# AislingGui/cst_captioning

Measured on AMD Instinct MI355X. Metric: SCST training captions/sec (whole node), MSR-VTT LSTM-attn at 1/2/4/8 MI355X, higher is better.
Workload: dtype bf16; 1 GPU; model=CaptionModel concat LSTM-512 (resnet+c3d+mfcc+category, V=10509, L=30), global_batch=1280, videos_per_gpu=64, seq_per_img=20, seq_len=30, parallelism=dp1, impl=hip, reward=gpu, mode=scst, params=20888845, dedupe_greedy=1, cuda_graph=1, grad_wire=fp32

## Files before the change

csrc/bindings.cpp:

```cpp
#include <torch/extension.h>

#include "engine.h"
#include "host/cider_host.h"
#include "host/metric_host.h"
#include "launchers.h"

namespace cst {

template <class T>
static at::Tensor to_tensor(const std::vector<T>& v, at::ScalarType st) {
  at::Tensor t = at::empty({(int64_t)v.size()}, at::TensorOptions().dtype(st));
  if (!v.empty()) std::memcpy(t.data_ptr(), v.data(), v.size() * sizeof(T));
  return t;
}

static std::map<std::string, at::Tensor> cider_build_tables(at::Tensor labels, at::Tensor start,
                                                            at::Tensor end, at::Tensor df_keys,
                                                            at::Tensor df_vals,
                                                            double log_ref_len, int64_t use_eos) {
  TORCH_CHECK(!labels.is_cuda(), "host builder takes CPU tensors");
  labels = labels.contiguous().to(at::kLong);
  start = start.contiguous().to(at::kLong);
  end = end.contiguous().to(at::kLong);
  df_keys = df_keys.contiguous().to(at::kLong);
// ... 254 lines not shown
          return py::cast(cst::reward_mix_score(hyps, hyp_video, cider_tables, tables,
                                                log_ref_len, use_eos, *weights));
        }
        TORCH_CHECK(tables.has_value(), "metric_score: tables must be given");
        TORCH_CHECK(!weights.has_value() && !cider_tables.has_value(),
                    "metric_score: weights / cider_tables go with metric mix only");
        return py::cast(cst::metric_score(metric, hyps, hyp_video, *tables, use_eos, exclude));
      },
      py::arg("metric"), py::arg("hyps"), py::arg("hyp_video"), py::arg("tables"),
      py::arg("use_eos"), py::arg("exclude") = py::none(), py::arg("cider_tables") = py::none(),
      py::arg("log_ref_len") = 0.0, py::arg("weights") = py::none(), py::arg("group") = 0,
      "Bleu_4 | ROUGE_L sentence scores on the GPU, or their weighted mix with CIDEr-D "
      "(metric mix; group = G >= 2: every row against the others of its pool of G); one "
      "launch, capturable");
  m.def(
      "metric_score_cpu",
      [](const std::string& metric, at::Tensor hyps, at::Tensor hyp_video,
         c10::optional<std::map<std::string, at::Tensor>> tables, int64_t use_eos,
         c10::optional<at::Tensor> exclude,
         c10::optional<std::map<std::string, at::Tensor>> cider_tables, double log_ref_len,
         c10::optional<std::vector<double>> weights, int64_t group) -> py::object {
        if (group != 0) {
          TORCH_CHECK(metric == "mix",
                      "metric_score_cpu: peer mode (group > 0) is metric mix, got ", metric);
          TORCH_CHECK(weights.has_value(), "metric_score_cpu: metric mix needs weights");
          TORCH_CHECK(!(exclude.has_value() && exclude->defined()),
                      "metric_score_cpu: peer mode (group > 0) takes no exclude");
          return py::cast(cst::peer_mix_score_cpu(hyps, cider_tables, log_ref_len, use_eos,
                                                  *weights, group));
        }
        TORCH_CHECK(!weights.has_value() && !cider_tables.has_value(),
                    "metric_score_cpu: weights / cider_tables go with peer mode (metric mix, "
                    "group > 0) only");
        TORCH_CHECK(tables.has_value(), "metric_score_cpu: tables must be given");
        return py::cast(cst::metric_score_cpu(metric, hyps, hyp_video, *tables, use_eos, exclude));
      },
      py::arg("metric"), py::arg("hyps"), py::arg("hyp_video"), py::arg("tables"),
      py::arg("use_eos"), py::arg("exclude") = py::none(), py::arg("cider_tables") = py::none(),
      py::arg("log_ref_len") = 0.0, py::arg("weights") = py::none(), py::arg("group") = 0);
  m.def("flat_adam_step", &cst::flat_adam_step, py::arg("p"), py::arg("g"), py::arg("m"),
        py::arg("v"), py::arg("partials"), py::arg("scal"), py::arg("skip"), py::arg("hyper"),
        py::arg("b1"), py::arg("b2"), py::arg("eps"), py::arg("clip"), py::arg("gscale"),
        py::arg("phase"), py::arg("shadow_meta"), py::arg("shadow_dst"),
        py::arg("ema") = py::none(), py::arg("ema_decay") = 0.0);
  m.def("refresh_shadows", &cst::refresh_shadows, py::arg("p"), py::arg("shadow_meta"),
        py::arg("shadow_dst"), py::arg("swap_with") = py::none());
  m.def("vocab_fwd_bench", &cst::vocab_fwd_bench);
  m.def("vgrad_colsum_bench", &cst::vgrad_colsum_bench);
  m.def("token_sort_bench", &cst::token_sort_bench);
  m.def("att_bench", &cst::att_bench);
  m.def("token_sort", &cst::token_sort);
  m.def("token_group_sum", &cst::token_group_sum);
  m.def("vocab_select", &cst::vocab_select);
  m.def("decode_step_test", &cst::decode_step_test);
  m.def("gemm_bf16_tuned", &cst::gemm_bf16_tuned, py::arg("out"), py::arg("a"), py::arg("ta"),
        py::arg("b"), py::arg("tb"), py::arg("n_cand") = 24);
  m.def("gemm_bf16_tuned_batched", &cst::gemm_bf16_tuned_batched, py::arg("out"), py::arg("a"),
        py::arg("ta"), py::arg("b"), py::arg("tb"), py::arg("n_cand") = 24);
  m.def("gemm_tuned_timings", &cst::gemm_tuned_timings);
  m.def("gemm_tuned_choices", &cst::gemm_tuned_choices);
  m.def("set_grad_events", &cst::set_grad_events);
  m.def("grad_event_wait", &cst::grad_event_wait);
  m.def("grad_event_record", &cst::grad_event_record);
  m.def("grad_event_count", &cst::grad_event_count);
  m.def("set_poll_bound", &cst::set_poll_bound,
        "polls of a bounded cross-workgroup wait before it gives up (tests: 0)");
  m.def("set_bwd_loop", &cst::set_bwd_loop,
        "reverse LSTM loop: 1 one persistent launch, row-read form (default); 2 persistent, "
        "K-split team GEMM; 0 one launch per step");
  m.def("lstm_bwd_loop_bench", &cst::lstm_bwd_loop_bench, py::arg("R"), py::arg("H"), py::arg("T"),
        py::arg("iters"), py::arg("phases"), py::arg("dbg") = 0,
        "persistent reverse loop alone on random operands: us per launch (+ phase stamps)");
  m.def("set_att_fuse", &cst::set_att_fuse,
        "attention backward fused into the reverse step (true, default) or a launch per step");
  m.def("device_errors", &cst::device_errors,
        "failed cross-workgroup hand-offs counted on the device (synchronous read)");
  m.def("reset_device_errors", &cst::reset_device_errors);
  m.def("att_mfma_fwd", &cst::att_mfma_fwd, py::arg("h"), py::arg("wq"), py::arg("P"),
        py::arg("wa"), py::arg("ba"), py::arg("gv"), py::arg("whole") = -1);
  m.def("beam_search", &cst::beam_search);
  m.def("featpool_forward", &cst::featpool_forward, py::arg("xs"), py::arg("ws"), py::arg("bs"),
        py::arg("drop_p"), py::arg("rng"), py::arg("idx") = py::none(), py::arg("C") = 1);
  m.def("featpool_forward16", &cst::featpool_forward16, py::arg("xs"), py::arg("ws"),
        py::arg("bs"), py::arg("drop_p"), py::arg("rng"), py::arg("idx") = py::none(),
        py::arg("C") = 1);
  m.def("scst_loss_forward", &cst::scst_loss_forward);
  m.def("cst_loss_forward", &cst::cst_loss_forward, py::arg("seq"), py::arg("lp"),
        py::arg("scores"), py::arg("bref"), py::arg("S"), py::arg("k"), py::arg("objective") = 0,
        py::arg("alpha") = 1.0, py::arg("cost_scale") = 1.0);
  m.def("scst_loss_backward", &cst::scst_loss_backward, py::arg("seq"), py::arg("reward"),
        py::arg("out"), py::arg("dloss"), py::arg("row_weight") = py::none());
  m.def("xe_loss_forward", &cst::xe_loss_forward);
  m.def("xe_loss_backward", &cst::xe_loss_backward);
  m.def("featpool_backward", &cst::featpool_backward, py::arg("dout"), py::arg("out"),
        py::arg("xs"), py::arg("ws"), py::arg("drop_p"), py::arg("outs"),
        py::arg("idx") = py::none(), py::arg("C") = 1);
  m.def("set_stamp_base", &cst::set_stamp_base);
  m.def("stamp_buffer", &cst::stamp_buffer);
  m.def("stamp_now", &cst::stamp_now);
  m.def("busy_copy", &cst::busy_copy,
        "stand-in for a collective's kernel: copying workgroups for a given time");
  m.def("wall_clock_khz", &cst::wall_clock_khz);
  m.def("vocab_x", &cst::vocab_x);
  m.def("att_mfma_phases", &cst::att_mfma_phases);
  m.def("wgrad_tn", &cst::wgrad_tn);
  m.def("wgrad_tn_colsum", &cst::wgrad_tn_colsum);
  m.def("wgrad_tn_rows", &cst::wgrad_tn_rows);
// ... 10 lines not shown
```

csrc/decoder_forward.cpp:

```cpp
#include "engine_internal.h"

namespace cst {
namespace {

struct Rollout {
  const at::Tensor &wx, &emb, &ptab, &whh, &wlog, &blog, &vgate;
  const int64_t vgate_div;
  const at::Tensor &labels, &bos;
  const int64_t R, T;
  const std::vector<int64_t>& modes;
  const double ss_prob, drop_p, temperature;
  const at::Tensor& rng;
  const bool save, want_xe, use_counts, use_unfinished;
  const std::vector<at::Tensor>& att;
  const int64_t cell;
  const std::vector<at::Tensor>&state0, &up;
  const bool store_exp, xe_rows;
  const c10::optional<at::Tensor>& lab_idx;
  bool has_att = false, have_labels = false, have_idx = false;
  int64_t H4 = 0, H = 0, E = 0, V = 0, L = 0, n_steps = 0, NL = 1;
  const uint16_t* PTAB = nullptr;
  AttOperands ao;
  UpperLayers upl;
  InitState s0;
// ... 221 lines not shown
    at::Tensor tgt_all = labels.narrow(1, 1, n_steps).t().contiguous();
    at::Tensor gx = at::empty({n_steps, R}, f32);
    stamp(STAMP_FWD_BEGIN, st);
    launch_lstm_step_fwd(LAB, L, PTAB, nullptr, nullptr, VG, VDIV, (int)R, (int)H, WHH,
                         h_buf(0, 0), c_buf(0, 0), hd_buf(0, 0), (int)H, (float)drop_p, RNG,
                         key(0, 0), gates_buf(0, 0), st, nullptr, (int)cell);
    stamp(STAMP_FWD_STEP0, st);
    for (int64_t t = 0; t < n_steps; ++t) {
      const bool next = t + 1 < n_steps;
      XeCell xc{};
      if (next)
        xc = XeCell{LAB + (t + 1), L, PTAB, c_buf(0, t), h_buf(0, t + 1), c_buf(0, t + 1),
                    hd_buf(0, t + 1), gates_buf(0, t + 1), (float)drop_p, key(0, t + 1),
                    (int)cell};
      char* pt = reinterpret_cast<char*>(part_all.data_ptr()) + t * pstep;
      launch_vocab_lstm_xe(hd_buf(0, t), (int)R, (int)H, W, blog.data_ptr<float>(), (int)V,
                           reinterpret_cast<uint16_t*>(logits16[t].data_ptr()), ldl, pt,
                           tgt_all.data_ptr<int64_t>() + t * R, RNG, h_buf(0, t), WHH, VG, VDIV,
                           next ? &xc : nullptr, st);
    }
    launch_vocab_combine(part_all.data_ptr(), n_vt, (int)(n_steps * R), lse.data_ptr<float>(),
                         nullptr, 0, nullptr, 0, gx.data_ptr<float>(), 1, nullptr, 0, SEL_GT_H,
                         0.f, RNG, 0, nullptr, 0, nullptr, st, nullptr, (int)R);
    at::Tensor gxt = gx.t();
    g_xe.copy_(gxt);
    g_sel.copy_(gxt.narrow(1, 0, T - 1));
    seq.copy_(labels.narrow(1, 1, T - 1));
    stamp(STAMP_FWD_END, st);
    return {seq, g_sel, g_xe, lse, logits16, HDs[0], Gs[0], Cs[0], Hs[0]};
  }

  std::vector<at::Tensor> run_steps() {
    const int64_t Bv = ao.Bv, C = ao.C, A = ao.A;
    stamp(STAMP_FWD_BEGIN, st);
    if (has_att) run_att(0);
    launch_lstm_step_fwd(have_labels ? LABR : TokRows(bos.data_ptr<int64_t>()), have_labels ? L : 1,
                         PTAB,
                         state0.empty() ? nullptr : reinterpret_cast<uint16_t*>(h0.data_ptr()),
                         state0.empty() ? nullptr : c0.data_ptr<float>(), VG, VDIV, (int)R, (int)H, WHH, h_buf(0, 0),
                         c_buf(0, 0), hd_buf(0, 0), (int)H, (float)drop_p, RNG, key(0, 0),
                         gates_buf(0, 0), st, nullptr, (int)cell, &sinit);
    for (int64_t l = 1; l < NL; ++l) upper_step(l, 0);
    bool conv_join = false;
    for (int64_t t = 0; t < n_steps; ++t) {
      const bool next = t + 1 < n_steps;
      uint16_t* hd = hd_buf(NL - 1, t);
      const uint16_t* vin = hd ? hd : h_buf(NL - 1, t);
      const bool choose = t < T - 1;
      const int mode = choose ? (int)modes[t] : SEL_GT_H;
      const int do_sample = choose && (mode == SEL_SAMPLE_H || mode == SEL_SS_H);
      const bool exp_t = save && store_exp && t > 0;
      const int vflags = do_sample | ((choose && mode == SEL_GREEDY_H) ? 2 : 0) | (exp_t ? 16 : 0);
      const TokRows tgt = (have_labels && t + 1 < L) ? LABR.col(t + 1) : TokRows();
      at::Tensor q_next;
      if (has_att && next) q_next = save ? q_all[t + 1] : q_tmp;
      AttMfmaArgs am{};
      if (att_mfma && next)
        am = AttMfmaArgs{h_buf(0, t), WHH + H4 * H, ao.pre.data_ptr<float>(), ao.wa.data_ptr<float>(),
                         ao.ba.data_ptr<float>(), reinterpret_cast<const uint16_t*>(gv16.data_ptr()),
                         (int)H, (int)A, (int)C, ao.CPAD, (int)H4, (int)vgate_div, (int)Bv,
                         reinterpret_cast<uint16_t*>(vg16.data_ptr()),
                         save ? alpha_all[t + 1].data_ptr<float>() : nullptr,
                         save ? q_next.data_ptr<float>() : nullptr, att_ep.data_ptr<float>(),
                         att_cnt.data_ptr<int>(),
                         save ? reinterpret_cast<uint16_t*>(u_all[t + 1].data_ptr()) : nullptr};
      if (att_mfma && next) am.whole = att_mfma_whole_default((int)C, (int)H);
      const bool q_tiles = has_att && !att_mfma;
      const int n_vt = launch_vocab_lstm_fwd(
          vin, (int)H, (int)R, (int)H, W, blog.data_ptr<float>(), (int)V,
          save ? reinterpret_cast<uint16_t*>(logits16[t].data_ptr()) : nullptr, ldl, part.data_ptr(),
          tgt, L, vflags, inv_temp, RNG, (int)t, h_buf(0, t), WHH, has_att ? nullptr : VG, VDIV,
          next ? reinterpret_cast<float*>(pre.data_ptr()) : nullptr, st, q_tiles ? (int)A : 0,
          q_tiles && next ? q_next.data_ptr<float>() : nullptr,
          exp_t ? lse[t - 1].data_ptr<float>() : nullptr, att_mfma && next ? &am : nullptr,
          pre16 ? 1 : 0);
      if (q_tiles && next)
        launch_att_fwd(ao.gv.data_ptr<float>(), ao.pre.data_ptr<float>(), q_next.data_ptr<float>(),
                       nullptr, ao.wa.data_ptr<float>(), ao.ba.data_ptr<float>(), (int)Bv,
                       (int)vgate_div, (int)C, (int)A, (int)H4, pre.data_ptr<float>(),
                       save ? alpha_all[t + 1].data_ptr<float>() : nullptr, st, 1,
                       ao.per_frame);
      CellLaunch cl{};
      if (next) {
        TORCH_CHECK(choose, "internal: a next step needs a chosen token");
        cl = CellLaunch{pre.data_ptr(), PTAB, c_buf(0, t), c_buf(0, t + 1),
                        h_buf(0, t + 1), hd_buf(0, t + 1), (int)H, gates_buf(0, t + 1), (int)H,
                        (float)drop_p, key(0, t + 1), (int)cell,
                        att_mfma ? reinterpret_cast<const uint16_t*>(vg16.data_ptr()) : nullptr,
                        pre16 ? 1 : 0};
      }
      launch_vocab_combine(part.data_ptr(), n_vt, (int)R, lse[t].data_ptr<float>(),
                             choose ? seq.data_ptr<int64_t>() + t : nullptr, T - 1,
                             choose ? g_sel.data_ptr<float>() + t : nullptr, T - 1,
                             want_xe ? g_xe.data_ptr<float>() + t : nullptr, T, tgt, L, mode,
                             (float)ss_prob, RNG, (int)t,
                             use_counts ? counts.data_ptr<int>() : nullptr, (int)(t + 1),
                             use_unfinished ? unfinished.data_ptr<uint8_t>() : nullptr, st,
                             next ? &cl : nullptr);
      if (save && store_exp && t == 0) {
        DeviceAux& aux = device_aux((int)wx.device().index());
        const hipStream_t cs = aux.side[1].stream();
        fork(aux.fwd_ev[0], st, cs);
        launch_vocab_exp_convert(reinterpret_cast<uint16_t*>(logits16[0].data_ptr()), ldl, (int)V,
                                 (int)R, lse[0].data_ptr<float>(), cs);
        (void)hipEventRecord(aux.fwd_ev[1], cs);
        conv_join = true;
      }
      if (next)
        for (int64_t l = 1; l < NL; ++l) upper_step(l, t + 1);
      if (t == 0) stamp(STAMP_FWD_STEP0, st);
    }
    if (conv_join)
      (void)hipStreamWaitEvent(st, device_aux((int)wx.device().index()).fwd_ev[1], 0);
    stamp(STAMP_FWD_END, st);
    std::vector<at::Tensor> out = {seq, g_sel, want_xe ? g_xe : at::Tensor(), lse};
    if (save) {
      out.push_back(logits16);
      out.push_back(HDs[NL - 1]);
      out.push_back(Gs[0]);
      out.push_back(Cs[0]);
      out.push_back(Hs[0]);
      if (has_att) {
        out.push_back(alpha_all);
        out.push_back(q_all);
// ... 36 lines not shown
```

csrc/dev_entries.cpp:

```cpp
#include "engine_internal.h"

namespace cst {

double lstm_bwd_loop_bench(int64_t R, int64_t H, int64_t T, int64_t iters, at::Tensor phases,
                           int64_t dbg) {
  TORCH_CHECK(lstm_bwd_loop_ok((int)R, (int)H, (int)T), "lstm_bwd_loop_bench: unsupported shape");
  auto dev = at::Device(at::kCUDA, at::hip::getCurrentHIPStream().device_index());
  auto f32 = at::TensorOptions().dtype(at::kFloat).device(dev);
  auto b16 = at::TensorOptions().dtype(at::kBFloat16).device(dev);
  at::Tensor dG = at::empty({T, R, 4 * H}, b16);
  at::Tensor whhT = (at::randn({H, 4 * H}, f32) * 0.05).to(at::kBFloat16);
  at::Tensor dh = at::randn({T, R, H}, f32) * 0.01;
  at::Tensor gates = at::rand({T, R, 4 * H}, f32).to(at::kBFloat16);
  at::Tensor c_all = at::randn({T, R, H}, f32);
  at::Tensor dc = at::empty({R, H}, f32);
  at::Tensor rng = at::zeros({2}, at::TensorOptions().dtype(at::kInt).device(dev));
  BwdLoopArgs la{};
  la.dG = reinterpret_cast<uint16_t*>(dG.data_ptr());
  la.whhT = reinterpret_cast<const uint16_t*>(whhT.data_ptr());
  la.dh = dh.data_ptr<float>();
  la.gates = reinterpret_cast<const uint16_t*>(gates.data_ptr());
  la.c_all = c_all.data_ptr<float>();
  la.dc_out = dc.data_ptr<float>();
  la.R = (int)R;
// ... 268 lines not shown
  const int vdiv = (int)(R / Bv), CP = C <= 8 ? 8 : 16;
  TORCH_CHECK(att_mfma_fwd_ok(vdiv, (int)C, (int)A, (int)H, 0), "att_mfma: unsupported shape");
  at::Tensor gv16 = at::zeros({Bv, 4 * H, CP}, h.options());
  gv16.narrow(2, 0, C).copy_(gv.transpose(1, 2));
  at::Tensor vg = at::empty({R, 4 * H}, h.options());
  at::Tensor alpha = at::empty({R, C}, P.options()), q = at::empty({R, A}, P.options());
  at::Tensor ep = at::empty({Bv, A / 64, 32, CP}, P.options());
  at::Tensor cnt = at::zeros({Bv}, P.options().dtype(at::kInt));
  AttMfmaArgs a{reinterpret_cast<const uint16_t*>(h.data_ptr()),
                reinterpret_cast<const uint16_t*>(wq.data_ptr()), P.data_ptr<float>(),
                wa.data_ptr<float>(), ba.data_ptr<float>(),
                reinterpret_cast<const uint16_t*>(gv16.data_ptr()), (int)H, (int)A, (int)C, CP,
                (int)(4 * H), vdiv, (int)Bv, reinterpret_cast<uint16_t*>(vg.data_ptr()),
                alpha.data_ptr<float>(), q.data_ptr<float>(), ep.data_ptr<float>(),
                cnt.data_ptr<int>()};
  a.whole = whole < 0 ? att_mfma_whole_default((int)C, (int)H) : (whole != 0 ? 1 : 0);
  launch_att_mfma_fwd(a, cur_stream());
  return {vg, alpha, q};
}

std::vector<at::Tensor> vocab_select(at::Tensor hd, at::Tensor wlog, at::Tensor blog,
                                     at::Tensor rng, int64_t mode, double temperature,
                                     int64_t step) {
  check_cuda(hd, "hd");
  check_cuda(wlog, "wlog");
  TORCH_CHECK(hd.scalar_type() == at::kBFloat16 && wlog.scalar_type() == at::kBFloat16 &&
                  blog.scalar_type() == at::kFloat, "bf16 hd / W, fp32 bias");
  TORCH_CHECK(mode == SEL_SAMPLE_H || mode == SEL_GREEDY_H, "mode: 1 sample, 2 greedy");
  const int64_t R = hd.size(0), H = hd.size(1), V = wlog.size(0);
  TORCH_CHECK(H % 64 == 0 && wlog.size(1) == H && blog.numel() == V, "shapes");
  auto dev = hd.device();
  const int n_vt = vocab_num_tiles((int)V);
  at::Tensor part = at::empty({(int64_t)n_vt * R * vocab_partial_bytes() / 4},
                              at::TensorOptions().dtype(at::kFloat).device(dev));
  at::Tensor tok = at::zeros({R, 1}, at::TensorOptions().dtype(at::kLong).device(dev));
  at::Tensor lse = at::empty({R}, at::TensorOptions().dtype(at::kFloat).device(dev));
  hipStream_t st = cur_stream();
  launch_vocab_fwd(reinterpret_cast<const uint16_t*>(hd.data_ptr()), (int)H, (int)R, (int)H,
                   reinterpret_cast<const uint16_t*>(wlog.data_ptr()), blog.data_ptr<float>(),
                   (int)V, nullptr, 0, part.data_ptr(), nullptr, 0, mode == SEL_SAMPLE_H ? 1 : 2,
                   (float)(1.0 / temperature), rng_ptr(rng), (int)step, st);
  launch_vocab_combine(part.data_ptr(), n_vt, (int)R, lse.data_ptr<float>(),
                       tok.data_ptr<int64_t>(), 1, nullptr, 0, nullptr, 0, nullptr, 0, (int)mode,
                       0.f, rng_ptr(rng), (int)step, nullptr, 0, nullptr, st);
  return {tok.view({R}), lse};
}

std::vector<at::Tensor> decode_step_test(at::Tensor hd, at::Tensor h, at::Tensor wlog,
                                         at::Tensor blog, at::Tensor whh, at::Tensor vgate,
                                         int64_t vdiv, at::Tensor tgt, at::Tensor eoff,
                                         int64_t save, int64_t mode, int64_t step, at::Tensor rng,
                                         at::Tensor ptab, at::Tensor c_prev, double drop_p,
                                         int64_t cell, int64_t eos, at::Tensor unfinished,
                                         double ss_prob) {
  check_cuda(hd, "hd");
  check_cuda(wlog, "wlog");
  const int64_t R = hd.size(0), H = hd.size(1), V = wlog.size(0);
  TORCH_CHECK(hd.scalar_type() == at::kBFloat16 && wlog.scalar_type() == at::kBFloat16 &&
                  hd.is_contiguous() && wlog.is_contiguous() && wlog.size(1) == H &&
                  blog.scalar_type() == at::kFloat && blog.numel() == V, "hd / wlog / blog");
  const bool lstm = whh.defined() && whh.numel() > 0;
  if (lstm)
    TORCH_CHECK(h.scalar_type() == at::kBFloat16 && h.is_contiguous() && h.sizes() == hd.sizes() &&
                    whh.scalar_type() == at::kBFloat16 && whh.is_contiguous() &&
                    whh.size(0) == 4 * H && whh.size(1) == H, "h / whh");
  const bool has_vg = vgate.defined() && vgate.numel() > 0;
  if (has_vg)
    TORCH_CHECK(vgate.scalar_type() == at::kFloat && vgate.is_contiguous() &&
                    vgate.size(0) * vdiv == R && vgate.size(1) == 4 * H, "vgate (R / vdiv, 4H)");
  const bool has_tgt = tgt.defined() && tgt.numel() > 0;
  if (has_tgt) TORCH_CHECK(tgt.scalar_type() == at::kLong && tgt.numel() == R, "tgt (R) int64");
  if (save == 2)
    TORCH_CHECK(eoff.defined() && eoff.scalar_type() == at::kFloat && eoff.numel() == R, "eoff (R)");
  const bool do_cell = ptab.defined() && ptab.numel() > 0;
  if (do_cell) {
    TORCH_CHECK(lstm, "the cell needs the recurrent part");
    check_cuda(ptab, "ptab");
    check_cuda(c_prev, "c_prev");
    TORCH_CHECK(ptab.scalar_type() == at::kHalf && ptab.size(0) == V && ptab.size(1) == 4 * H &&
                    c_prev.scalar_type() == at::kFloat && c_prev.numel() == R * H,
                "ptab (V, 4H) fp16 / c_prev (R, H) fp32");
  }
  const bool has_unf = unfinished.defined() && unfinished.numel() > 0;
  if (has_unf)
    TORCH_CHECK(unfinished.is_cuda() && unfinished.scalar_type() == at::kByte &&
                    unfinished.numel() == R, "unfinished (R) uint8");
  auto dev = hd.device();
  auto f32 = at::TensorOptions().dtype(at::kFloat).device(dev);
  auto bf = at::TensorOptions().dtype(at::kBFloat16).device(dev);
  const int64_t ldl = (V + 63) / 64 * 64;
  at::Tensor part = at::empty({(int64_t)vocab_part_slots((int)V) * R * vocab_partial_bytes() / 4}, f32);
  at::Tensor saved = save ? at::zeros({R, ldl}, at::TensorOptions()
                                                    .dtype(save == 2 ? at::kBFloat16 : at::kHalf)
                                                    .device(dev))
                          : at::Tensor();
  at::Tensor pre = lstm ? at::zeros({R, 4 * H}, f32) : at::Tensor();
  at::Tensor lse = at::empty({R}, f32), gsel = at::zeros({R}, f32), gxe = at::zeros({R}, f32);
  at::Tensor tok = at::zeros({R}, at::TensorOptions().dtype(at::kLong).device(dev));
  at::Tensor h_out, c_out, hdrop, gates;
  if (do_cell) {
    h_out = at::zeros({R, H}, bf);
    c_out = at::zeros({R, H}, f32);
    hdrop = at::zeros({R, H}, bf);
    gates = at::zeros({R, 4 * H}, bf);
  }
  const int cps = combine_count_ints_per_step();
  at::Tensor counts = at::zeros({3 * cps}, at::TensorOptions().dtype(at::kInt).device(dev));
  if (eos == 1) counts.narrow(0, cps, 1).fill_(1);
  int* CNT = eos ? counts.data_ptr<int>() : nullptr;
  hipStream_t st = cur_stream();
  const int flags = (mode == SEL_SAMPLE_H || mode == SEL_SS_H ? 1 : 0) |
                    (mode == SEL_GREEDY_H ? 2 : 0) | (save == 2 ? 16 : 0);
  const int64_t* TG = has_tgt ? tgt.data_ptr<int64_t>() : nullptr;
  uint8_t* UNF = has_unf ? unfinished.data_ptr<uint8_t>() : nullptr;
  const int n = launch_vocab_lstm_fwd(
      reinterpret_cast<const uint16_t*>(hd.data_ptr()), (int)H, (int)R, (int)H,
      reinterpret_cast<const uint16_t*>(wlog.data_ptr()), blog.data_ptr<float>(), (int)V,
      save ? reinterpret_cast<uint16_t*>(saved.data_ptr()) : nullptr, ldl, part.data_ptr(), TG, 1,
      flags, 1.f, rng_ptr(rng), (int)step,
      lstm ? reinterpret_cast<const uint16_t*>(h.data_ptr()) : nullptr,
      lstm ? reinterpret_cast<const uint16_t*>(whh.data_ptr()) : nullptr,
      has_vg ? vgate.data_ptr<float>() : nullptr, (int)vdiv, lstm ? pre.data_ptr<float>() : nullptr,
      st, 0, nullptr, save == 2 ? eoff.data_ptr<float>() : nullptr, nullptr);
  CellLaunch cl{};
  if (do_cell)
    cl = CellLaunch{pre.data_ptr<float>(), reinterpret_cast<const uint16_t*>(ptab.data_ptr()),
                    c_prev.data_ptr<float>(), c_out.data_ptr<float>(),
                    reinterpret_cast<uint16_t*>(h_out.data_ptr()),
                    reinterpret_cast<uint16_t*>(hdrop.data_ptr()), (int)H,
                    reinterpret_cast<uint16_t*>(gates.data_ptr()), (int)H, (float)drop_p,
                    (int)step + 1, (int)cell, nullptr, 0};
  launch_vocab_combine(part.data_ptr(), n, (int)R, lse.data_ptr<float>(), tok.data_ptr<int64_t>(),
                       1, gsel.data_ptr<float>(), 1, has_tgt ? gxe.data_ptr<float>() : nullptr, 1,
                       TG, 1, (int)mode, (float)ss_prob, rng_ptr(rng), (int)step, CNT, 2, UNF, st,
                       do_cell ? &cl : nullptr);
  return {lse, tok, gsel, gxe, saved, pre, at::full({1}, n, at::TensorOptions().dtype(at::kLong)),
          h_out, c_out, hdrop, gates, counts};
}

std::vector<at::Tensor> token_sort(at::Tensor toks, int64_t V) {
  check_cuda(toks, "toks");
  TORCH_CHECK(toks.scalar_type() == at::kLong, "int64 token ids");
  const int64_t N = toks.numel();
  auto i32 = at::TensorOptions().dtype(at::kInt).device(toks.device());
  at::Tensor ws = at::empty({2 * V + 1}, i32), stok = at::empty({N}, i32), srow = at::empty({N}, i32);
  launch_token_sort(toks.data_ptr<int64_t>(), (int)N, (int)V, ws.data_ptr<int>(),
                    stok.data_ptr<int>(), srow.data_ptr<int>(), cur_stream());
  return {stok, srow};
}

at::Tensor token_group_sum(at::Tensor x, at::Tensor toks, int64_t V) {
  check_cuda(toks, "toks");
  TORCH_CHECK(x.is_cuda() && x.scalar_type() == at::kBFloat16 && x.dim() == 2 &&
                  x.stride(1) == 1 && x.stride(0) >= x.size(1) &&
                  reinterpret_cast<uintptr_t>(x.data_ptr()) % 16 == 0,
              "x: (N, C) bf16, unit column stride, 16-byte aligned");
  TORCH_CHECK(toks.scalar_type() == at::kLong && toks.numel() == x.size(0), "toks: (N) int64");
  const int64_t N = toks.numel(), C = x.size(1);
  auto i32 = at::TensorOptions().dtype(at::kInt).device(toks.device());
  at::Tensor ws = at::empty({2 * V + 1}, i32), stok = at::empty({N}, i32), srow = at::empty({N}, i32);
  at::Tensor S = at::empty({V, C}, x.options());
  at::Tensor S64 = at::empty({V, C}, x.options().dtype(at::kDouble));
  hipStream_t st = cur_stream();
  launch_token_sort(toks.data_ptr<int64_t>(), (int)N, (int)V, ws.data_ptr<int>(),
                    stok.data_ptr<int>(), srow.data_ptr<int>(), st);
  launch_token_long_zero(ws.data_ptr<int>(), (int)V, (int)C, S64.data_ptr<double>(), st);
  launch_token_group_sum(reinterpret_cast<const uint16_t*>(x.data_ptr()), (int)C, x.stride(0),
                         stok.data_ptr<int>(), srow.data_ptr<int>(), (int)N, ws.data_ptr<int>(),
                         (int)V, reinterpret_cast<uint16_t*>(S.data_ptr()), S64.data_ptr<double>(),
                         st);
  return S;
}

std::vector<at::Tensor> vgrad_fold(at::Tensor E, at::Tensor lse, at::Tensor y_sel,
                                   at::Tensor dg_sel, at::Tensor labels, at::Tensor dg_xe,
                                   int64_t V, int64_t zero_off, at::Tensor hd, at::Tensor wlog,
                                   at::Tensor blog, at::Tensor fix_total, bool forward_x,
                                   at::Tensor X) {
  check_cuda(E, "E");
  check_cuda(lse, "lse");
  TORCH_CHECK(E.scalar_type() == at::kBFloat16 && E.dim() == 3, "vgrad_fold: E (n, R, ldl) bf16");
  const int64_t n = E.size(0), R = E.size(1), ldl = E.size(2), NR = n * R;
  TORCH_CHECK(NR > 0 && V > 0 && V <= ldl && lse.scalar_type() == at::kFloat && lse.dim() == 2 &&
                  lse.size(0) == n && lse.size(1) == R,
              "vgrad_fold: V <= ldl, lse (n, R) fp32");
  auto in_vocab = [&](const at::Tensor& t) { return t.max().item<int64_t>() < V; };
  const bool has_sel = dg_sel.defined() && dg_sel.numel() > 0;
  const bool has_xe = dg_xe.defined() && dg_xe.numel() > 0;
  int64_t T_sel = 0;
  if (has_sel) {
// ... 128 lines not shown
```

csrc/engine.h:

```cpp
#pragma once
#include <torch/extension.h>

#include <map>
#include <string>
#include <vector>

namespace cst {

std::vector<at::Tensor> decoder_forward(at::Tensor wx, at::Tensor emb, at::Tensor ptab,
                                        at::Tensor whh, at::Tensor wlog,
                                        at::Tensor blog, at::Tensor vgate, int64_t vgate_div,
                                        at::Tensor labels, at::Tensor bos, int64_t R, int64_t T,
                                        std::vector<int64_t> modes, double ss_prob,
                                        double drop_p, double temperature, at::Tensor rng,
                                        bool save, bool want_xe, bool use_counts,
                                        bool use_unfinished, std::vector<at::Tensor> att,
                                        int64_t cell, std::vector<at::Tensor> state0,
                                        std::vector<at::Tensor> up, bool store_exp,
                                        bool xe_rows, c10::optional<at::Tensor> lab_idx);
std::vector<at::Tensor> decoder_backward(at::Tensor wx, at::Tensor wlog, at::Tensor emb,
                                         at::Tensor lse, at::Tensor logits16,
                                         at::Tensor hdrop_all, at::Tensor gates_all,
                                         at::Tensor c_all, at::Tensor h_all, at::Tensor seq,
                                         at::Tensor labels, at::Tensor toks, at::Tensor dg_sel,
// ... 57 lines not shown
std::vector<at::Tensor> xe_loss_forward(at::Tensor labels, at::Tensor lp, int64_t off);
at::Tensor xe_loss_backward(at::Tensor cnt, at::Tensor out, at::Tensor dloss, int64_t T);
at::Tensor scst_loss_backward(at::Tensor seq, at::Tensor reward, at::Tensor out,
                              at::Tensor dloss, c10::optional<at::Tensor> row_weight);
at::Tensor cider_score(at::Tensor hyps, at::Tensor hyp_video, std::map<std::string, at::Tensor> t,
                       double log_ref_len, int64_t use_eos, bool clipped,
                       c10::optional<at::Tensor> exclude, int64_t group);
at::Tensor bleu_stats(at::Tensor hyps, at::Tensor hyp_video, std::map<std::string, at::Tensor> t);
std::vector<at::Tensor> meteor_stats(at::Tensor hyps, at::Tensor hyp_video,
                                     std::map<std::string, at::Tensor> t, at::Tensor stem_ids,
                                     c10::optional<at::Tensor> exclude);
at::Tensor metric_score(const std::string& metric, at::Tensor hyps, at::Tensor hyp_video,
                        std::map<std::string, at::Tensor> t, int64_t use_eos,
                        c10::optional<at::Tensor> exclude);
std::vector<at::Tensor> reward_mix_score(
    at::Tensor hyps, at::Tensor hyp_video,
    c10::optional<std::map<std::string, at::Tensor>> cider_tables,
    c10::optional<std::map<std::string, at::Tensor>> sent_tables, double log_ref_len,
    int64_t use_eos, std::vector<double> weights);
std::vector<at::Tensor> peer_mix_score(at::Tensor hyps,
                                       c10::optional<std::map<std::string, at::Tensor>> df,
                                       double log_ref_len, int64_t use_eos,
                                       std::vector<double> weights, int64_t group);
at::Tensor flat_adam_step(at::Tensor p, at::Tensor g, at::Tensor m, at::Tensor v,
                          at::Tensor partials, at::Tensor scal, at::Tensor skip, at::Tensor hyper,
                          double b1, double b2, double eps, double clip, double gscale,
                          int64_t phase, at::Tensor shadow_meta,
                          std::vector<at::Tensor> shadow_dst, c10::optional<at::Tensor> ema,
                          double ema_decay);
void refresh_shadows(at::Tensor p, at::Tensor shadow_meta, std::vector<at::Tensor> shadow_dst,
                     c10::optional<at::Tensor> swap_with);

double lstm_bwd_loop_bench(int64_t R, int64_t H, int64_t T, int64_t iters, at::Tensor phases,
                           int64_t dbg);
double vocab_fwd_bench(at::Tensor hd, at::Tensor wlog, at::Tensor blog, at::Tensor tgt,
                       int64_t flags, bool save, int64_t iters, int64_t variant);
double vgrad_colsum_bench(at::Tensor E, at::Tensor alpha, int64_t V, int64_t iters);
double token_sort_bench(at::Tensor toks, int64_t V, int64_t iters);
double att_bench(at::Tensor gv, at::Tensor P, at::Tensor q, at::Tensor wa, at::Tensor ba,
                 int64_t R, int64_t which, int64_t iters);
at::Tensor att_mfma_phases(at::Tensor gv, at::Tensor P, at::Tensor wa, at::Tensor ba, int64_t R);
std::vector<at::Tensor> att_mfma_fwd(at::Tensor h, at::Tensor wq, at::Tensor P, at::Tensor wa,
                                     at::Tensor ba, at::Tensor gv,
                                     int64_t whole);
std::vector<at::Tensor> vocab_select(at::Tensor hd, at::Tensor wlog, at::Tensor blog,
                                     at::Tensor rng, int64_t mode, double temperature,
                                     int64_t step);
std::vector<at::Tensor> decode_step_test(at::Tensor hd, at::Tensor h, at::Tensor wlog,
                                         at::Tensor blog, at::Tensor whh, at::Tensor vgate,
                                         int64_t vdiv, at::Tensor tgt, at::Tensor eoff,
                                         int64_t save, int64_t mode, int64_t step, at::Tensor rng,
                                         at::Tensor ptab, at::Tensor c_prev, double drop_p,
                                         int64_t cell, int64_t eos, at::Tensor unfinished,
                                         double ss_prob);
std::vector<at::Tensor> token_sort(at::Tensor toks, int64_t V);
at::Tensor token_group_sum(at::Tensor x, at::Tensor toks, int64_t V);
std::vector<at::Tensor> vgrad_fold(at::Tensor E, at::Tensor lse, at::Tensor y_sel,
                                   at::Tensor dg_sel, at::Tensor labels, at::Tensor dg_xe,
                                   int64_t V, int64_t zero_off, at::Tensor hd, at::Tensor wlog,
                                   at::Tensor blog, at::Tensor fix_total, bool forward_x,
                                   at::Tensor X);
at::Tensor vgrad_rows(at::Tensor alpha, at::Tensor hd, int64_t ldhs, at::Tensor dhd);
at::Tensor vgrad_colsum(at::Tensor E, at::Tensor alpha, int64_t V);
at::Tensor video_gate_grad(at::Tensor dG, int64_t vdiv, int64_t G4);
at::Tensor wgrad_tn(at::Tensor A, at::Tensor B, int64_t M, int64_t N, int64_t K);
void wgrad_tn_rows(at::Tensor A, at::Tensor B, int64_t M, int64_t N, int64_t K, at::Tensor out,
                   at::Tensor rmap);
std::vector<at::Tensor> wgrad_tn_colsum(at::Tensor A, at::Tensor B, at::Tensor al, int64_t M,
                                        int64_t N, int64_t K);
void busy_copy(at::Tensor buf, int64_t blocks, double us, int64_t stream);

}
```

csrc/kernels/vocab.hip:

```cpp
#include "gemm_tile.h"
#include "lstm_gemm.h"
#include "att_mfma.h"
#include "vocab_common.h"
#include "../launchers.h"

namespace cst {

constexpr int VT_V = 128;
constexpr int EXP_STAGE_LD = VT_V + 8;
__host__ __device__ constexpr int exp_stage_off(int BN) { return 4 * BN * 32; }
__host__ __device__ constexpr int epilogue_lds_bytes(int BN) {
  return exp_stage_off(BN) + BN * EXP_STAGE_LD * 2;
}
struct GroupStat {
  float m, s, zkey, zlogit;
  int zidx, xidx;
  float xt, pad;
};

#define VOCAB_TR_PARAMS                                                                     \
  const uint16_t *__restrict__ hd, int ldh, int R, int H, const uint16_t *__restrict__ W,    \
      const float *__restrict__ bias, int V, uint16_t *__restrict__ logits16, int64_t ldl,   \
      VocabPartial *__restrict__ part, TokRows tgt, int64_t tgt_stride,                     \
      int flags, float inv_temp, const uint32_t *__restrict__ rng, int step,                 \
      const float *__restrict__ eoff
#define VOCAB_TR_ARGS \
  hd, ldh, R, H, W, bias, V, logits16, ldl, part, tgt, tgt_stride, flags, inv_temp, rng, step, eoff

template <int BN, int STAGES, bool TOPK = false>
__device__ __forceinline__ void vocab_tr_block(int bid, char* lds, VOCAB_TR_PARAMS) {
  using TL = Tile<VT_V, BN, STAGES>;
  constexpr int TM = TL::TM, TN = TL::TN;
  static_assert(TM == 2, "lane owns 32 vocab entries per row");
  const int n_vt = (V + VT_V - 1) / VT_V, n_rt = (R + BN - 1) / BN;
  const int b = xcd_remap(bid, n_vt * n_rt);
  const int vt = b / n_rt, rt = b % n_rt;
  const int v0 = vt * VT_V, r0 = rt * BN;
  const int nk = H / 64;
  const int lane = threadIdx.x & 63, w = threadIdx.x >> 6, wr = w >> 1, wc = w & 1;
  const int half = lane >> 5;
  const int vb = v0 + wr * TL::WM + 4 * half;

  float pb[TM][16];
#pragma unroll
  for (int i = 0; i < TM; ++i)
#pragma unroll
    for (int q = 0; q < 4; ++q) {
      const int v = vb + 32 * i + 8 * q;
      if (v + 4 <= V) {
        const float4 x = *reinterpret_cast<const float4*>(bias + v);
        pb[i][4 * q] = x.x, pb[i][4 * q + 1] = x.y, pb[i][4 * q + 2] = x.z, pb[i][4 * q + 3] = x.w;
      } else {
#pragma unroll
        for (int e = 0; e < 4; ++e) pb[i][4 * q + e] = v + e < V ? bias[v + e] : -INFINITY;
      }
    }
  int tg[TN];
  float ec[TN];
#pragma unroll
  for (int j = 0; j < TN; ++j) {
    const int r = min(r0 + wc * TL::WN + 32 * j + (lane & 31), R - 1);
    tg[j] = tgt.p != nullptr ? (int)tgt.at(r, tgt_stride) : -1;
    ec[j] = eoff != nullptr ? eoff[r] : 0.f;
  }

  f32x16 acc[TM][TN];
  {
    DmaSrc<VT_V / 32> a;
    DmaSrc<BN / 32> bsrc;
    a.r0 = a.r1 = make_rsrc(W, (int64_t)V * H * 2);
    a.ksplit = nk;
#pragma unroll
    for (int i = 0; i < VT_V / 32; ++i) {
      const int row = dma_row(w, i, lane);
      a.voff0[i] = min(v0 + row, V - 1) * H * 2 + dma_chunk(row, lane) * 16;
      a.voff1[i] = a.voff0[i];
    }
    bsrc.r0 = bsrc.r1 = make_rsrc(hd, (int64_t)R * ldh * 2);
    bsrc.ksplit = nk;
#pragma unroll
// ... 39 lines not shown
          for (int p = 0; p < VF_TOPK_MAXK; ++p) {
            if (p < K && cv > tv[p]) {
              const float a = tv[p];
              const int b = ti[p];
              tv[p] = cv, ti[p] = ci;
              cv = a, ci = b;
            }
          }
        }
      float2* tk = reinterpret_cast<float2*>(lds + exp_stage_off(BN));
#pragma unroll
      for (int p = 0; p < VF_TOPK_MAXK; ++p)
        tk[(g * BN + row_l) * VF_TOPK_MAXK + p] = make_float2(tv[p], __int_as_float(ti[p]));
    } else if ((flags & VF_SAVE_F32) && logits16 != nullptr && r < R) {
      float* dst = reinterpret_cast<float*>(logits16) + (int64_t)r * ldl;
#pragma unroll
      for (int i = 0; i < TM; ++i)
#pragma unroll
        for (int q = 0; q < 4; ++q) {
          const int v = vb + 32 * i + 8 * q;
          if (v + 4 <= V) {
            *reinterpret_cast<float4*>(dst + v) =
                make_float4(x[i][4 * q], x[i][4 * q + 1], x[i][4 * q + 2], x[i][4 * q + 3]);
          } else {
#pragma unroll
            for (int e = 0; e < 4; ++e)
              if (v + e < V) dst[v + e] = x[i][4 * q + e];
          }
        }
    } else if (logits16 != nullptr && r < R && !(flags & VF_EXP)) {
      uint16_t* et = reinterpret_cast<uint16_t*>(lds + exp_stage_off(BN)) + row_l * EXP_STAGE_LD;
#pragma unroll
      for (int i = 0; i < TM; ++i)
#pragma unroll
        for (int q = 0; q < 4; ++q) {
          const int vl = vb - v0 + 32 * i + 8 * q;
          uint2 pk;
          pk.x = (uint32_t)f2h(x[i][4 * q]) | ((uint32_t)f2h(x[i][4 * q + 1]) << 16);
          pk.y = (uint32_t)f2h(x[i][4 * q + 2]) | ((uint32_t)f2h(x[i][4 * q + 3]) << 16);
          *reinterpret_cast<uint2*>(et + vl) = pk;
        }
    }

    float m = -INFINITY;
#pragma unroll
    for (int i = 0; i < TM; ++i)
#pragma unroll
      for (int k = 0; k < 16; ++k) m = fmaxf(m, x[i][k]);
    const float msafe = m == -INFINITY ? 0.f : m;
    const float ml = msafe * L2E;
    float ew[TM][16];
    float s = 0.f;
#pragma unroll
    for (int i = 0; i < TM; ++i)
#pragma unroll
      for (int k = 0; k < 16; ++k) {
        ew[i][k] = __builtin_amdgcn_exp2f(fmaf(x[i][k], L2E, -ml));
        s += ew[i][k];
      }
    if ((flags & VF_EXP) && logits16 != nullptr && r < R) {
      const float f = __builtin_amdgcn_exp2f((msafe - ec[j]) * L2E);
      uint16_t* et = reinterpret_cast<uint16_t*>(lds + exp_stage_off(BN)) + row_l * EXP_STAGE_LD;
#pragma unroll
      for (int i = 0; i < TM; ++i)
#pragma unroll
        for (int q = 0; q < 4; ++q) {
          const int vl = vb - v0 + 32 * i + 8 * q;
          uint2 pk;
          pk.x = (uint32_t)f2bf(ew[i][4 * q] * f) | ((uint32_t)f2bf(ew[i][4 * q + 1] * f) << 16);
          pk.y = (uint32_t)f2bf(ew[i][4 * q + 2] * f) | ((uint32_t)f2bf(ew[i][4 * q + 3] * f) << 16);
          *reinterpret_cast<uint2*>(et + vl) = pk;
        }
    }

    GroupStat st;
    st.m = m;
    st.s = s;
    st.pad = 0.f;
    st.xidx = 0x7fffffff;
    if (flags & VF_ARGMAX) {
#pragma unroll
      for (int i = 0; i < TM; ++i)
#pragma unroll
        for (int k = 0; k < 16; ++k) {
          const int v = vb + 32 * i + 8 * (k >> 2) + (k & 3);
          st.xidx = min(st.xidx, x[i][k] == m ? v : 0x7fffffff);
        }
    }
    st.xt = -INFINITY;
    if (tgt.p != nullptr) {
      const int d = tg[j] - vb;
      const bool mine = d >= 0 && d < 32 * TM && (d & 4) == 0;
      const int kk = mine ? (d >> 5) * 16 + ((d >> 3) & 3) * 4 + (d & 3) : -1;
#pragma unroll
      for (int i = 0; i < TM; ++i)
#pragma unroll
        for (int k = 0; k < 16; ++k) st.xt = (i * 16 + k == kk) ? x[i][k] : st.xt;
    }
    st.zkey = -INFINITY;
    st.zlogit = 0.f;
    st.zidx = 0x7fffffff;
    if (flags & VF_SAMPLE) {
      const float wl = msafe * inv_temp * L2E, wsc = inv_temp * L2E;
      float sw = s;
      if (!temp1) {
        sw = 0.f;
#pragma unroll
        for (int i = 0; i < TM; ++i)
#pragma unroll
          for (int k = 0; k < 16; ++k) {
            ew[i][k] = __builtin_amdgcn_exp2f(fmaf(x[i][k], wsc, -wl));
            sw += ew[i][k];
          }
      }
      const uint32_t rr = (uint32_t)min(r, R - 1);
      const uint32_t seed = rng_seed(rng, RNG_SLOT_SAMPLE);
      const uint32_t key = mix32(seed ^ mix32(rr * 0x9E3779B1u + (uint32_t)step * 0x85EBCA77u) ^
                                 (uint32_t)(vt * 4 + g) * 0xC2B2AE3Du);
      const float u = ((float)(key >> 8) + 0.5f) * (1.0f / 16777216.0f);
      const float tm = u * sw;
      float cum = 0.f, cl = 0.f;
      int cand = -1;
#pragma unroll
      for (int i = 0; i < TM; ++i)
#pragma unroll
        for (int k = 0; k < 16; ++k) {
          const float wv = ew[i][k];
          cum += wv;
          const bool hit = cand < 0 && cum >= tm && wv > 0.f;
          cand = hit ? vb + 32 * i + 8 * (k >> 2) + (k & 3) : cand;
          cl = hit ? x[i][k] : cl;
        }
      if (sw > 0.f && cand >= 0) {
        const uint32_t key2 = mix32(key ^ 0x68E31DA4u);
        const float u2 = ((float)(key2 >> 8) + 0.5f) * (1.0f / 16777216.0f);
        st.zkey = msafe * inv_temp + __logf(sw) - __logf(-__logf(u2));
        st.zidx = cand;
        st.zlogit = cl;
      }
    }
    gs[g * BN + row_l] = st;
  }
  __syncthreads();
  if (threadIdx.x < BN) {
    const int row_l = threadIdx.x, r = r0 + row_l;
    if (r < R) {
      GroupStat a = gs[row_l];
#pragma unroll
      for (int q = 1; q < 4; ++q) {
        const GroupStat c = gs[q * BN + row_l];
        const float M = fmaxf(a.m, c.m);
        a.s = (a.m == -INFINITY ? 0.f : a.s * __expf(a.m - M)) +
              (c.m == -INFINITY ? 0.f : c.s * __expf(c.m - M));
        if (c.m > a.m || (c.m == a.m && c.xidx < a.xidx)) a.xidx = c.xidx;
        a.m = M;
        if (c.zkey > a.zkey || (c.zkey == a.zkey && c.zidx < a.zidx)) {
          a.zkey = c.zkey;
          a.zidx = c.zidx;
          a.zlogit = c.zlogit;
        }
        a.xt = fmaxf(a.xt, c.xt);
      }
      VocabPartial p;
      p.m = a.m;
      p.s = a.s;
      p.zval = a.zkey;
      p.zlogit = a.zlogit;
      p.zidx = a.zidx;
      p.xidx = a.xidx;
      p.xtgt = a.xt;
      p.pad = 0.f;
      part[(int64_t)vt * R + r] = p;
      if (TOPK && (flags & VF_TOPK)) {
        const int K = vf_topk_k(flags);
        const float2* tk = reinterpret_cast<const float2*>(lds + exp_stage_off(BN));
        int hd4[4] = {0, 0, 0, 0};
        float2* dst = reinterpret_cast<float2*>(logits16) + ((int64_t)vt * R + r) * K;
        for (int k = 0; k < K; ++k) {
          float bvv = -INFINITY;
          int bii = 0x7fffffff, bq = 0;
#pragma unroll
          for (int q = 0; q < 4; ++q) {
            const float2 c = hd4[q] < K ? tk[(q * BN + row_l) * VF_TOPK_MAXK + hd4[q]]
                                        : make_float2(-INFINITY, __int_as_float(0x7fffffff));
            const int ci = __float_as_int(c.y);
            if (c.x > bvv || (c.x == bvv && ci < bii)) bvv = c.x, bii = ci, bq = q;
          }
#pragma unroll
          for (int q = 0; q < 4; ++q) hd4[q] += q == bq ? 1 : 0;
          dst[k] = make_float2(bvv, __int_as_float(bii));
        }
// ... 633 lines not shown
```

csrc/launchers.h:

```cpp
#pragma once
#include <hip/hip_runtime.h>
#include <stdint.h>

namespace cst {

struct TokRows {
  const int64_t* p;
  const int64_t* idx;
  int64_t n;
  __host__ __device__ TokRows(const int64_t* p_ = nullptr, const int64_t* idx_ = nullptr,
                              int64_t n_ = 0)
      : p(p_), idx(idx_), n(n_) {}
  __host__ __device__ int64_t at(int r, int64_t stride) const {
    int64_t row = r;
    if (idx != nullptr) {
      row = idx[r];
      row = row < 0 ? 0 : (row >= n ? n - 1 : row);
    }
    return p[row * stride];
  }
  __host__ __device__ TokRows col(int64_t c) const {
    return TokRows(p != nullptr ? p + c : nullptr, idx, n);
  }
};
// ... 61 lines not shown
  const float* ng_val = nullptr;
  float log_ref_len = 0.f;
};
struct MixSentArgs {
  int Nv = 0;
  const int32_t *vid_ref_off = nullptr, *ref_len = nullptr, *vid_ng_off = nullptr;
  const int64_t* ng_key = nullptr;
  const int32_t *ng_cnt = nullptr, *ref_tok_off = nullptr, *ref_tok = nullptr;
};
void launch_reward_mix(const int64_t* hyps, int T, const int64_t* hyp_video, int N,
                       const MixCiderArgs& c, const MixSentArgs& s, int use_eos, float w_c,
                       float w_b, float w_r, float* out, float* parts, hipStream_t stream);

void launch_peer_mix(const int64_t* hyps, int T, int G, int B, const int64_t* ht_keys,
                     const float* ht_vals, uint32_t ht_cap, float log_ref_len, int use_eos,
                     float w_c, float w_b, float w_r, float* out, float* parts,
                     hipStream_t stream);

void launch_bleu_stats(const int64_t* hyps, int T, const int64_t* hyp_video, int N, int Nv,
                       const int32_t* vid_ref_off, const int32_t* ref_len,
                       const int32_t* vid_ng_off, const int64_t* ng_key, const int32_t* ng_cnt,
                       int32_t* out, hipStream_t stream);
void launch_meteor_stats(const int64_t* hyps, int T, const int64_t* hyp_video, int N, int Nv,
                         const int32_t* vid_ref_off, const int32_t* ref_tok_off,
                         const int32_t* ref_tok, const int32_t* ref_stem,
                         const int32_t* stem_ids, int V, const int64_t* exclude,
                         int32_t* out_stats, double* out_score, hipStream_t stream);

enum ShadowKind : int { SHADOW_PLAIN = 0, SHADOW_GATES_IH = 1, SHADOW_GATES_HH = 2 };
constexpr int SHADOW_MAX_SEGS = 12;
struct ShadowSeg {
  int64_t off, n;
  int kind;
  int cols;
  int H, E;
  uint16_t* dst;
  uint16_t* dst2;
  int ld2;
  int slots;
};
struct ShadowSegs {
  ShadowSeg s[SHADOW_MAX_SEGS];
  int n;
};
void launch_flat_adam(float* p, const float* g, float* m, float* v, int64_t n, float* partials,
                      const bool* skip, float* scal, float* hyper, float b1, float b2,
                      float eps, float clip, float gscale, int phase, const ShadowSegs& ss,
                      float* ema, float one_minus_d, hipStream_t stream);
void launch_shadow_refresh(const float* p, const ShadowSegs& ss, hipStream_t stream);
void launch_swap_refresh(float* p, float* q, int64_t n, const ShadowSegs& ss,
                         hipStream_t stream);

enum SelModeHost : int { SEL_GT_H = 0, SEL_SAMPLE_H = 1, SEL_GREEDY_H = 2, SEL_SS_H = 3 };
constexpr int VF_TOPK_H = 32;
int vocab_num_tiles(int V);
void launch_vocab_fwd_variant(int variant, const uint16_t* hd, int ldh, int R, int H,
                              const uint16_t* W, const float* bias, int V, uint16_t* logits16,
                              int64_t ldl, void* part, const int64_t* tgt, int64_t tgt_stride,
                              int flags, float inv_temp, const uint32_t* rng, int step,
                              hipStream_t stream);
int vocab_partial_bytes();
void launch_vocab_fwd(const uint16_t* hd, int ldh, int R, int H, const uint16_t* W,
                      const float* bias,
                      int V, uint16_t* logits16, int64_t ldl, void* part, const int64_t* tgt,
                      int64_t tgt_stride, int flags, float inv_temp, const uint32_t* rng,
                      int step, hipStream_t stream,
                      const float* eoff = nullptr);
struct CellLaunch {
  const void* pre;
  const uint16_t* ptab;
  const float* c_prev;
  float* c_out;
  uint16_t* h_out;
  uint16_t* hdrop_out;
  int ldh;
  uint16_t* gates_out;
  int H;
  float drop_p;
  int step;
  int cell;
  const uint16_t* vg16;
  int pre_half;
};
struct AttFwdArgs {
  const float* gv;
  const float* pre;
  const float* q;
  const int* q_rowmap;
  const float* wa;
  const float* ba;
  int wa_ld, ba_ld, vdiv, ngroups, C, A, G4;
  float* vg_out;
  float* alpha_out;
  int accumulate;
};
struct AttMfmaArgs {
  const uint16_t* h;
  const uint16_t* wq;
  const float* P;
  const float* wa;
  const float* ba;
  const uint16_t* gv16;
  int H, A, C, CP, G4, vdiv, Bv;
  uint16_t* vg_out;
  float* alpha_out;
  float* q_out;
// ... 290 lines not shown
```

Measured before the change: 415,700 captions/s.

## Skip target-logit gather when unused and streamline vocab epilogue selects

The decoder step no longer passes the target token pointer to the fused vocab kernel when neither the XE loss nor GT/scheduled-sampling selection needs it, so SCST sampling steps skip the target-logit extraction. The vocab epilogue replaces the per-element compare loops for argmax, target pick and sampled-token pick with a count-then-binary-select tree (pick32), and packs the exp2 argument FMAs into two-wide vector ops. This is meant to cut VALU instruction count and register churn in the per-tile epilogue. The sampling pick changes from first hit with positive weight to counting prefix sums below the threshold, which can differ in edge cases with zero weights.

```diff
diff --git a/csrc/bindings.cpp b/csrc/bindings.cpp
--- a/csrc/bindings.cpp
+++ b/csrc/bindings.cpp
@@ -330,7 +330,11 @@
   m.def("token_sort", &cst::token_sort);
   m.def("token_group_sum", &cst::token_group_sum);
   m.def("vocab_select", &cst::vocab_select);
-  m.def("decode_step_test", &cst::decode_step_test);
+  m.def("decode_step_test", &cst::decode_step_test, py::arg("hd"), py::arg("h"), py::arg("wlog"),
+        py::arg("blog"), py::arg("whh"), py::arg("vgate"), py::arg("vdiv"), py::arg("tgt"),
+        py::arg("eoff"), py::arg("save"), py::arg("mode"), py::arg("step"), py::arg("rng"),
+        py::arg("ptab"), py::arg("c_prev"), py::arg("drop_p"), py::arg("cell"), py::arg("eos"),
+        py::arg("unfinished"), py::arg("ss_prob"), py::arg("want_xe") = true);
   m.def("gemm_bf16_tuned", &cst::gemm_bf16_tuned, py::arg("out"), py::arg("a"), py::arg("ta"),
         py::arg("b"), py::arg("tb"), py::arg("n_cand") = 24);
   m.def("gemm_bf16_tuned_batched", &cst::gemm_bf16_tuned_batched, py::arg("out"), py::arg("a"),
diff --git a/csrc/decoder_forward.cpp b/csrc/decoder_forward.cpp
--- a/csrc/decoder_forward.cpp
+++ b/csrc/decoder_forward.cpp
@@ -297,6 +297,7 @@
       const bool exp_t = save && store_exp && t > 0;
       const int vflags = do_sample | ((choose && mode == SEL_GREEDY_H) ? 2 : 0) | (exp_t ? 16 : 0);
       const TokRows tgt = (have_labels && t + 1 < L) ? LABR.col(t + 1) : TokRows();
+      const TokRows tgt_x = vocab_step_reads_target(want_xe, choose, mode) ? tgt : TokRows();
       at::Tensor q_next;
       if (has_att && next) q_next = save ? q_all[t + 1] : q_tmp;
       AttMfmaArgs am{};
@@ -314,7 +315,7 @@
       const int n_vt = launch_vocab_lstm_fwd(
           vin, (int)H, (int)R, (int)H, W, blog.data_ptr<float>(), (int)V,
           save ? reinterpret_cast<uint16_t*>(logits16[t].data_ptr()) : nullptr, ldl, part.data_ptr(),
-          tgt, L, vflags, inv_temp, RNG, (int)t, h_buf(0, t), WHH, has_att ? nullptr : VG, VDIV,
+          tgt_x, L, vflags, inv_temp, RNG, (int)t, h_buf(0, t), WHH, has_att ? nullptr : VG, VDIV,
           next ? reinterpret_cast<float*>(pre.data_ptr()) : nullptr, st, q_tiles ? (int)A : 0,
           q_tiles && next ? q_next.data_ptr<float>() : nullptr,
           exp_t ? lse[t - 1].data_ptr<float>() : nullptr, att_mfma && next ? &am : nullptr,
diff --git a/csrc/dev_entries.cpp b/csrc/dev_entries.cpp
--- a/csrc/dev_entries.cpp
+++ b/csrc/dev_entries.cpp
@@ -344,7 +344,7 @@
                                          int64_t save, int64_t mode, int64_t step, at::Tensor rng,
                                          at::Tensor ptab, at::Tensor c_prev, double drop_p,
                                          int64_t cell, int64_t eos, at::Tensor unfinished,
-                                         double ss_prob) {
+                                         double ss_prob, bool want_xe) {
   check_cuda(hd, "hd");
   check_cuda(wlog, "wlog");
   const int64_t R = hd.size(0), H = hd.size(1), V = wlog.size(0);
@@ -404,11 +404,13 @@
   const int flags = (mode == SEL_SAMPLE_H || mode == SEL_SS_H ? 1 : 0) |
                     (mode == SEL_GREEDY_H ? 2 : 0) | (save == 2 ? 16 : 0);
   const int64_t* TG = has_tgt ? tgt.data_ptr<int64_t>() : nullptr;
+  const bool xe = has_tgt && want_xe;
+  const int64_t* TGX = vocab_step_reads_target(xe, true, (int)mode) ? TG : nullptr;
   uint8_t* UNF = has_unf ? unfinished.data_ptr<uint8_t>() : nullptr;
   const int n = launch_vocab_lstm_fwd(
       reinterpret_cast<const uint16_t*>(hd.data_ptr()), (int)H, (int)R, (int)H,
       reinterpret_cast<const uint16_t*>(wlog.data_ptr()), blog.data_ptr<float>(), (int)V,
-      save ? reinterpret_cast<uint16_t*>(saved.data_ptr()) : nullptr, ldl, part.data_ptr(), TG, 1,
+      save ? reinterpret_cast<uint16_t*>(saved.data_ptr()) : nullptr, ldl, part.data_ptr(), TGX, 1,
       flags, 1.f, rng_ptr(rng), (int)step,
       lstm ? reinterpret_cast<const uint16_t*>(h.data_ptr()) : nullptr,
       lstm ? reinterpret_cast<const uint16_t*>(whh.data_ptr()) : nullptr,
@@ -423,11 +425,11 @@
                     reinterpret_cast<uint16_t*>(gates.data_ptr()), (int)H, (float)drop_p,
                     (int)step + 1, (int)cell, nullptr, 0};
   launch_vocab_combine(part.data_ptr(), n, (int)R, lse.data_ptr<float>(), tok.data_ptr<int64_t>(),
-                       1, gsel.data_ptr<float>(), 1, has_tgt ? gxe.data_ptr<float>() : nullptr, 1,
+                       1, gsel.data_ptr<float>(), 1, xe ? gxe.data_ptr<float>() : nullptr, 1,
                        TG, 1, (int)mode, (float)ss_prob, rng_ptr(rng), (int)step, CNT, 2, UNF, st,
                        do_cell ? &cl : nullptr);
   return {lse, tok, gsel, gxe, saved, pre, at::full({1}, n, at::TensorOptions().dtype(at::kLong)),
-          h_out, c_out, hdrop, gates, counts};
+          h_out, c_out, hdrop, gates, counts, part};
 }
 
 std::vector<at::Tensor> token_sort(at::Tensor toks, int64_t V) {
diff --git a/csrc/engine.h b/csrc/engine.h
--- a/csrc/engine.h
+++ b/csrc/engine.h
@@ -133,7 +133,7 @@
                                          int64_t save, int64_t mode, int64_t step, at::Tensor rng,
                                          at::Tensor ptab, at::Tensor c_prev, double drop_p,
                                          int64_t cell, int64_t eos, at::Tensor unfinished,
-                                         double ss_prob);
+                                         double ss_prob, bool want_xe = true);
 std::vector<at::Tensor> token_sort(at::Tensor toks, int64_t V);
 at::Tensor token_group_sum(at::Tensor x, at::Tensor toks, int64_t V);
 std::vector<at::Tensor> vgrad_fold(at::Tensor E, at::Tensor lse, at::Tensor y_sel,
diff --git a/csrc/kernels/vocab.hip b/csrc/kernels/vocab.hip
--- a/csrc/kernels/vocab.hip
+++ b/csrc/kernels/vocab.hip
@@ -26,6 +26,33 @@
       const float *__restrict__ eoff
 #define VOCAB_TR_ARGS \
   hd, ldh, R, H, W, bias, V, logits16, ldl, part, tgt, tgt_stride, flags, inv_temp, rng, step, eoff
+
+__device__ __forceinline__ float sel32(bool c, float hi, float lo) { return c ? hi : lo; }
+__device__ __forceinline__ float pick32(const float (&x)[2][16], int n) {
+  const bool b0 = n & 1, b1 = n & 2, b2 = n & 4, b3 = n & 8, b4 = n & 16;
+  float a[16], b[8], c[4];
+#pragma unroll
+  for (int p = 0; p < 8; ++p) {
+    a[p] = sel32(b0, x[0][2 * p + 1], x[0][2 * p]);
+    a[8 + p] = sel32(b0, x[1][2 * p + 1], x[1][2 * p]);
+  }
+#pragma unroll
+  for (int p = 0; p < 8; ++p) b[p] = sel32(b1, a[2 * p + 1], a[2 * p]);
+#pragma unroll
+  for (int p = 0; p < 4; ++p) c[p] = sel32(b2, b[2 * p + 1], b[2 * p]);
+  return sel32(b4, sel32(b3, c[3], c[2]), sel32(b3, c[1], c[0]));
+}
+typedef float f32x2 __attribute__((ext_vector_type(2)));
+__device__ __forceinline__ void exp2_args(float (&a)[16], const float (&x)[16], float sc, float off) {
+#pragma unroll
+  for (int k = 0; k < 16; k += 2) {
+    const f32x2 r = __builtin_elementwise_fma(f32x2{x[k], x[k + 1]}, f32x2{sc, sc}, f32x2{off, off});
+    a[k] = r.x, a[k + 1] = r.y;
+  }
+}
+__device__ __forceinline__ int lane_vocab(int vb, int n) {
+  return vb + 32 * (n >> 4) + 8 * ((n >> 2) & 3) + (n & 3);
+}
 
 template <int BN, int STAGES, bool TOPK = false>
 __device__ __forceinline__ void vocab_tr_block(int bid, char* lds, VOCAB_TR_PARAMS) {
@@ -171,12 +198,14 @@
     float ew[TM][16];
     float s = 0.f;
 #pragma unroll
-    for (int i = 0; i < TM; ++i)
+    for (int i = 0; i < TM; ++i) {
+      exp2_args(ew[i], x[i], L2E, -ml);
 #pragma unroll
       for (int k = 0; k < 16; ++k) {
-        ew[i][k] = __builtin_amdgcn_exp2f(fmaf(x[i][k], L2E, -ml));
+        ew[i][k] = __builtin_amdgcn_exp2f(ew[i][k]);
         s += ew[i][k];
       }
+    }
     if ((flags & VF_EXP) && logits16 != nullptr && r < R) {
       const float f = __builtin_amdgcn_exp2f((msafe - ec[j]) * L2E);
       uint16_t* et = reinterpret_cast<uint16_t*>(lds + exp_stage_off(BN)) + row_l * EXP_STAGE_LD;
@@ -198,23 +227,19 @@
     st.pad = 0.f;
     st.xidx = 0x7fffffff;
     if (flags & VF_ARGMAX) {
-#pragma unroll
-      for (int i = 0; i < TM; ++i)
-#pragma unroll
-        for (int k = 0; k < 16; ++k) {
-          const int v = vb + 32 * i + 8 * (k >> 2) + (k & 3);
-          st.xidx = min(st.xidx, x[i][k] == m ? v : 0x7fffffff);
-        }
+      int n = 32;
+#pragma unroll
+      for (int i = TM - 1; i >= 0; --i)
+#pragma unroll
+        for (int k = 15; k >= 0; --k) n = x[i][k] == m ? 16 * i + k : n;
+      st.xidx = n < 32 ? lane_vocab(vb, n) : 0x7fffffff;
     }
     st.xt = -INFINITY;
     if (tgt.p != nullptr) {
       const int d = tg[j] - vb;
       const bool mine = d >= 0 && d < 32 * TM && (d & 4) == 0;
-      const int kk = mine ? (d >> 5) * 16 + ((d >> 3) & 3) * 4 + (d & 3) : -1;
-#pragma unroll
-      for (int i = 0; i < TM; ++i)
-#pragma unroll
-        for (int k = 0; k < 16; ++k) st.xt = (i * 16 + k == kk) ? x[i][k] : st.xt;
+      const float xk = pick32(x, (d >> 5) * 16 + ((d >> 3) & 3) * 4 + (d & 3));
+      st.xt = mine ? xk : -INFINITY;
     }
     st.zkey = -INFINITY;
     st.zlogit = 0.f;
@@ -225,12 +250,14 @@
       if (!temp1) {
         sw = 0.f;
 #pragma unroll
-        for (int i = 0; i < TM; ++i)
+        for (int i = 0; i < TM; ++i) {
+          exp2_args(ew[i], x[i], wsc, -wl);
 #pragma unroll
           for (int k = 0; k < 16; ++k) {
-            ew[i][k] = __builtin_amdgcn_exp2f(fmaf(x[i][k], wsc, -wl));
+            ew[i][k] = __builtin_amdgcn_exp2f(ew[i][k]);
             sw += ew[i][k];
           }
+        }
       }
       const uint32_t rr = (uint32_t)min(r, R - 1);
       const uint32_t seed = rng_seed(rng, RNG_SLOT_SAMPLE);
@@ -238,24 +265,21 @@
                                  (uint32_t)(vt * 4 + g) * 0xC2B2AE3Du);
       const float u = ((float)(key >> 8) + 0.5f) * (1.0f / 16777216.0f);
       const float tm = u * sw;
-      float cum = 0.f, cl = 0.f;
-      int cand = -1;
+      float cum = 0.f;
+      int n = 0;
 #pragma unroll
       for (int i = 0; i < TM; ++i)
 #pragma unroll
         for (int k = 0; k < 16; ++k) {
-          const float wv = ew[i][k];
-          cum += wv;
-          const bool hit = cand < 0 && cum >= tm && wv > 0.f;
-          cand = hit ? vb + 32 * i + 8 * (k >> 2) + (k & 3) : cand;
-          cl = hit ? x[i][k] : cl;
-        }
-      if (sw > 0.f && cand >= 0) {
+          cum += ew[i][k];
+          n += cum < tm ? 1 : 0;
+        }
+      if (sw > 0.f && n < 32) {
         const uint32_t key2 = mix32(key ^ 0x68E31DA4u);
         const float u2 = ((float)(key2 >> 8) + 0.5f) * (1.0f / 16777216.0f);
         st.zkey = msafe * inv_temp + __logf(sw) - __logf(-__logf(u2));
-        st.zidx = cand;
-        st.zlogit = cl;
+        st.zidx = lane_vocab(vb, n);
+        st.zlogit = pick32(x, n);
       }
     }
     gs[g * BN + row_l] = st;
diff --git a/csrc/launchers.h b/csrc/launchers.h
--- a/csrc/launchers.h
+++ b/csrc/launchers.h
@@ -137,6 +137,9 @@
                          hipStream_t stream);
 
 enum SelModeHost : int { SEL_GT_H = 0, SEL_SAMPLE_H = 1, SEL_GREEDY_H = 2, SEL_SS_H = 3 };
+inline bool vocab_step_reads_target(bool want_xe, bool choose, int mode) {
+  return want_xe || (choose && (mode == SEL_GT_H || mode == SEL_SS_H));
+}
 constexpr int VF_TOPK_H = 32;
 int vocab_num_tiles(int V);
 void launch_vocab_fwd_variant(int variant, const uint16_t* hd, int ldh, int R, int H,
```

Result: faster. 425,200 captions/s, median of 6 (+2.3%).
